# BosonHBC/BHRayTracer

Hardware: AMD Instinct MI355X
Metric: Mrays/s (closest-hit + any-hit rays per second), with wall-clock per frame (higher is better)
Workload: dtype f32

## Files before the change

bhraytracer_amd/csrc/device_state.h:

```cpp
#pragma once

namespace bhrt {

template <class T> struct DevBuf {
    T *p = nullptr;
    size_t n = 0;
    DevBuf() = default;
    DevBuf(const DevBuf &) = delete;
    DevBuf &operator=(const DevBuf &) = delete;
    DevBuf(DevBuf &&o) noexcept : p(o.p), n(o.n) { o.p = nullptr; o.n = 0; }
    DevBuf &operator=(DevBuf &&o) noexcept
    {
        if (this != &o) { Free(); p = o.p; n = o.n; o.p = nullptr; o.n = 0; }
        return *this;
    }
    ~DevBuf() { Free(); }
    int Reserve(size_t want)
    {
        if (n >= want) return BHRT_OK;
        Free();
        HIP_CHECK(hipMalloc(&p, want * sizeof(T)));
        n = want;
        return BHRT_OK;
    }
// ... 88 lines not shown
    int photon_exact = 0;
    uint32_t *d_knn = nullptr;
    DevBuf<uint32_t> d_sel;
    struct PendingTimer { int e0, e1; double *acc; };
    std::vector<PendingTimer> ev_pending;
    std::vector<int> ev_free;
    DevBuf<DPhoton> d_photons;
    uint32_t n_photons = 0;
    std::vector<HostPhoton> h_photons;
    DevBuf<float> d_ph_frames;
    DevBuf<float4> d_ph_hot, d_ph_cold, d_ph_dbox;
    PhotonMapDev pm;
    DevBuf<unsigned long long> d_scr;
    uint32_t scr_lanes = 0;
    uint32_t heavy_cap = 0;
    DevBuf<uint32_t> d_heavy;
    DevBuf<uint32_t> d_long;
    DevBuf<uint32_t> d_cell_of, d_gorder, d_rank_of, d_keys_out;
    DevBuf<uint8_t> d_sort_temp;
    size_t sort_temp_bytes = 0;
    DevBuf<uint32_t> d_n_heavy;
    PinnedBuf<uint32_t> h_n_heavy;
    DevBuf<uint32_t> d_cells, d_tile_sums;
    struct Knobs {
        int stream_waves = -1;
        bool fused_camera = true;
        bool no_slow_queue = false;
        bool debug_slow = false, debug_gather = false, debug_drain = false;
        bool balance_host = false;
        int frame_cap = 0;
        int gather_lane_budget = 0;
        bool gather_counting_sort = false;
        bool shadow_overlap = true;
        int gather_stats = 0;
        void FromEnv()
        {
            if (const char *e = getenv("BHRT_STREAM_WAVES")) stream_waves = atoi(e);
            if (const char *e = getenv("BHRT_FUSED_CAMERA")) fused_camera = atoi(e) != 0;
            no_slow_queue = getenv("BHRT_NO_SLOW_QUEUE") != nullptr;
            debug_slow = getenv("BHRT_DEBUG_SLOW") != nullptr; debug_gather = getenv("BHRT_DEBUG_GATHER") != nullptr; debug_drain = getenv("BHRT_DEBUG_DRAIN") != nullptr;
            if (const char *e = getenv("BHRT_PHOTON_BALANCE_HOST")) balance_host = atoi(e) != 0;
            if (const char *e = getenv("BHRT_GATHER_COUNTING_SORT")) gather_counting_sort = atoi(e) != 0;
            if (const char *e = getenv("BHRT_SHADOW_OVERLAP")) shadow_overlap = atoi(e) != 0;
        }
    } knobs;
    uint64_t pass_hint_key = 0;
    uint32_t pass_hint = 0;
    uint64_t frames_seen_key = 0;
    double frames_seen = 0;
    size_t frame_px = 0;
    DevBuf<uint8_t> d_frame_rgb;
    DevBuf<float> d_frame_rad, d_frame_var;
    DevBuf<uint32_t> d_frame_cnt;
    DevBuf<uint8_t> d_ad;
    DevBuf<uint8_t> d_dn;
    size_t api_cap = 0;
    DevBuf<float> d_api_f;
    DevBuf<int32_t> d_api_i;
};

void DestroyDeviceState(DeviceState *d)
{
    if (!d) return;
    if (d->device >= 0) (void)hipSetDevice(d->device);
    delete d;
}

}
```

bhraytracer_amd/csrc/kernels.hip:

```cpp
#include <hip/hip_runtime.h>

#include <stdlib.h>
#include <string.h>

#include <algorithm>
#include <type_traits>
#include <chrono>
#include <string>
#include <vector>

#include "bhrt.h"
#include "denoise.h"
#include "device_color24.h"
#include "device_photon.h"
#include "photon_host.h"
#include "scene_internal.h"

namespace bhrt {

#define HIP_CHECK(expr)                                                                                        \
    do {                                                                                                       \
        hipError_t e_ = (expr);                                                                                \
        if (e_ != hipSuccess) {                                                                                \
            SetError(std::string(#expr) + ": " + hipGetErrorString(e_));                                       \
// ... 183 lines not shown
{
    const uint32_t lane = __lane_id();
    const uint64_t lt = (1ull << lane) - 1ull;
    const uint64_t m0 = __ballot(cls == RC_HEAVY), m1 = __ballot(cls == RC_MEDIUM), m2 = __ballot(cls == RC_LIGHT), m3 = __ballot(cls == RC_MESH);
    uint32_t base = 0;
    if (lane < 4) {
        const uint64_t mk = lane == 0 ? m0 : (lane == 1 ? m1 : (lane == 2 ? m2 : m3));
        const uint32_t c = (uint32_t)__popcll(mk);
        if (c) base = atomicAdd(&cnt->cls[lane][shard].v, c);
    }
    const uint32_t wshard = shard;
    const uint32_t b0 = __shfl(base, 0), b1 = __shfl(base, 1), b2 = __shfl(base, 2), b3 = __shfl(base, 3);
    if (cls != RC_NONE) {
        const uint64_t mm = cls == RC_HEAVY ? m0 : (cls == RC_MEDIUM ? m1 : (cls == RC_LIGHT ? m2 : m3));
        const uint32_t pos = (cls == RC_HEAVY ? b0 : (cls == RC_MEDIUM ? b1 : (cls == RC_LIGHT ? b2 : b3))) + (uint32_t)__popcll(mm & lt);
        if (pos < ord.shard_cap) ord.idx[((size_t)cls * BHRT_ORDER_SHARDS + wshard) * ord.shard_cap + pos] = i;
        else atomicOr(&cnt->overflow.v, 8u);
    }
}
__device__ inline uint32_t shading_class(uint32_t meta, const Hit &hit)
{
    const uint32_t kind = meta & 15u;
    const bool is_hit = hit.node >= 0;
    bool heavy = false;
    if (is_hit) {
        if (kind == RK_CAMERA) heavy = true;
        else if (kind == RK_GI) heavy = fabsf(hit.t) > BHRT_BIAS;
        else if (kind == RK_REFR_IN) heavy = hit.front != 0;
        else heavy = true;
    }
    return heavy ? RC_HEAVY : ((kind == RK_REFR_IN && is_hit) ? RC_MEDIUM : RC_LIGHT);
}

struct SlowQueue {
    RayQueue q;
    uint32_t cap;
};
constexpr uint32_t kSlowCap = 1u << 16;
template <bool kPark, bool kCamera, bool kMeshes = true>
__global__ void __launch_bounds__(kBlock) k_trace_closest(DevScene S, PassInfo P, RayQueue q, uint32_t n, int uniform_side, HitBuf h, RayOrder ord, Counters *cnt,
                                                          SlowQueue slow )
{
    __shared__ bhrt_bvh_node nodelet[(kPark || !kMeshes) ? 1 : BHRT_LDS_NODES];
    const uint32_t i = blockIdx.x * blockDim.x + threadIdx.x;
    bool active = i < n;
    V3 o = v3(0, 0, 0), d = v3(0, 0, 1);
    uint32_t meta = 0;
    if (active) fetch_ray<kCamera>(S, P, q, i, o, d, meta);
    const bool has_meta = kCamera || q.meta;
    const int side = has_meta ? (int)((meta >> 4) & 3u) : uniform_side;
    const bool dead = has_meta && (meta & 15u) == RK_DEAD;
    Hit hit;
    uint32_t key = 0;
    bool is_slow = false;
    int parked = trace_closest<kMeshes>(S, o, d, side, hit, active && !dead, (kPark || !kMeshes) ? nullptr : nodelet, 0, kPark, kPark ? &key : nullptr,
                                        (uint16_t *)nullptr, 0, BHRT_LDS_NODES, kCamera, kPark ? &is_slow : nullptr);
    if (kPark && parked >= 0 && is_slow && slow.cap) {
        const uint32_t k = atomicAdd(&cnt->n_slow.v, 1u);
        if (k < slow.cap) {
            slow.q.ox[k] = o.x; slow.q.oy[k] = o.y; slow.q.oz[k] = o.z; slow.q.dx[k] = d.x; slow.q.dy[k] = d.y; slow.q.dz[k] = d.z;
            slow.q.frame[k] = kCamera ? i : q.frame[i];
            slow.q.meta[k] = meta;
            slow.q.rng_ctr[k] = (kCamera || (meta & 15u) == RK_GI) ? 0u : q.rng_ctr[i];
            active = false;
            parked = -1;
        }
    }
    if (active) { h.t[i] = hit.t; h.node[i] = hit.node; h.prim[i] = hit.prim; h.front[i] = hit.front | ((parked + 1) << 8); }
    if (kPark && parked >= 0) {
        ord.park_key[i] = key;
        if (!kCamera) ord.park_rank[i] = atomicAdd(&ord.park_bucket[key], 1u);
    }
    if (!ord.idx) return;
    uint32_t cls = RC_NONE;
    if (active && !dead) cls = parked >= 0 ? (uint32_t)RC_MESH : shading_class(meta, hit);
    file_ray(cls, i, (i >> 10) & (BHRT_ORDER_SHARDS - 1) , ord, cnt);
}
__device__ inline bool parked_entry(const RayOrder &ord, uint32_t b, uint32_t *s_seg, uint32_t &i, uint32_t first_entry = 0 )
{
    __syncthreads();
    if (threadIdx.x < 64) {
        const uint32_t l = threadIdx.x;
        const uint32_t a = l <= BHRT_ORDER_SHARDS ? ord.mesh_start[l] : 0xffffffffu;
        const uint32_t n_le = (uint32_t)__popcll(__ballot(l < BHRT_ORDER_SHARDS && a <= b));
        if (l == 0) *s_seg = n_le - 1;
    }
    __syncthreads();
    if (b >= ord.mesh_start[BHRT_ORDER_SHARDS]) return false;
    const uint32_t seg = *s_seg;
    const uint32_t local = (b - ord.mesh_start[seg]) * kBlock + first_entry + threadIdx.x;
    const bool active = local < ord.mesh_count[seg];
    i = active ? ord.idx[((size_t)RC_MESH * BHRT_ORDER_SHARDS + seg) * ord.shard_cap + local] : 0xffffffffu;
    return true;
}
#ifndef BHRT_XCD_LOCAL
#define BHRT_XCD_LOCAL 0
#endif
__device__ inline bool xcd_slice(uint32_t b, uint32_t nb, uint32_t &slice)
{
    slice = b;
#if BHRT_XCD_LOCAL
    constexpr uint32_t G = BHRT_XCD_LOCAL, span = 8 * G;
    const uint32_t chunk = b / span, in = b % span;
    if ((chunk + 1) * span <= nb) slice = chunk * span + (in & 7u) * G + (in >> 3);
#endif
    return b < nb;
}
__global__ void __launch_bounds__(kBlock) k_park_scatter(RayOrder ord)
{
    __shared__ uint32_t s_seg;
    uint32_t i;
    for (uint32_t b = blockIdx.x; parked_entry(ord, b, &s_seg, i); b += gridDim.x)
        if (i != 0xffffffffu) ord.park_sorted[ord.park_bucket[ord.park_key[i]] + ord.park_rank[i]] = i;
}
constexpr uint32_t kMeshNodelet = 256;
#ifndef BHRT_MESH_BLOCK
#define BHRT_MESH_BLOCK 64
#endif
constexpr int kMeshBlock = BHRT_MESH_BLOCK;
template <bool kCamera, int kPath, bool kLS = false>
__global__ void __launch_bounds__(kCamera ? kBlock : kMeshBlock, kPath == 1 ? 6 : 4 ) k_trace_mesh(DevScene S, PassInfo P, RayQueue q, HitBuf h, RayOrder ord, Counters *cnt)
{
    typedef typename std::conditional<kPath == 2, uint32_t, uint16_t>::type PathT;
    constexpr int kTB = kCamera ? kBlock : kMeshBlock;
    __shared__ bhrt_bvh_node nodelet[kPath ? 1 : kMeshNodelet];
    __shared__ PathT path[kPath ? 33 * kTB : 1];
    __shared__ uint32_t s_seg;
    bool active;
    uint32_t i;
    uint32_t slice;
    if (kCamera) {
        if (!xcd_slice(blockIdx.x, ord.mesh_start[BHRT_ORDER_SHARDS], slice)) return;
        if (!parked_entry(ord, slice, &s_seg, i)) return;
        active = i != 0xffffffffu;
        if (!active) i = 0;
    } else {
        const uint32_t total = ord.mesh_count[BHRT_ORDER_SHARDS];
        if (!xcd_slice(blockIdx.x, (total + kTB - 1) / kTB, slice)) return;
        const uint32_t k = slice * kTB + threadIdx.x;
        active = k < total;
        i = active ? ord.park_sorted[k] : 0u;
    }
    V3 o = v3(0, 0, 0), d = v3(0, 0, 1);
    uint32_t meta = 0;
    Hit hit = {BHRT_BIGFLOAT, -1, -1, 1};
    int start = 0;
    if (active) {
        fetch_ray<kCamera>(S, P, q, i, o, d, meta);
        hit.t = h.t[i]; hit.node = h.node[i]; hit.prim = h.prim[i];
        const int fw = h.front[i];
        hit.front = fw & 0xff;
        start = (fw >> 8) - 1;
    }
    trace_closest<true, PathT, kLS>(S, o, d, (int)((meta >> 4) & 3u), hit, active, kPath ? nullptr : nodelet, active ? start : S.n_nodes, false, nullptr,
                               kPath ? path + threadIdx.x : (PathT *)nullptr, kTB, kMeshNodelet);
    if (active) { h.t[i] = hit.t; h.node[i] = hit.node; h.prim[i] = hit.prim; h.front[i] = hit.front; }
    if (kCamera) file_ray(active ? shading_class(meta, hit) : (uint32_t)RC_NONE, i, slice & (BHRT_ORDER_SHARDS - 1), ord, cnt);
}
#ifndef BHRT_STREAM_REFILL
#define BHRT_STREAM_REFILL 32
#endif
constexpr int kStreamRefill = BHRT_STREAM_REFILL;
#ifndef BHRT_STREAM_OCC
#define BHRT_STREAM_OCC 6
#endif
#ifdef BHRT_DEBUG_DRAIN
__device__ unsigned long long g_stream_t[4];
#endif
#ifdef BHRT_DEBUG_STREAM
__device__ unsigned long long g_stream_dbg[8];
#endif
template <int kPath, bool kLS = false>
__global__ void __launch_bounds__(64, kPath == 1 ? BHRT_STREAM_OCC : (BHRT_STREAM_OCC < 5 ? BHRT_STREAM_OCC : 5) ) k_trace_mesh_stream(DevScene S, RayQueue q, HitBuf h, RayOrder ord, Counters *cnt)
{
    typedef typename std::conditional<kPath == 2, uint32_t, uint16_t>::type PathT;
    __shared__ PathT path[33 * 64];
    const uint32_t total = ord.mesh_count[BHRT_ORDER_SHARDS];
    const uint32_t lane = threadIdx.x;
    PathT *stack = path + lane;
    bool have = false, pending = false, exhausted = false;
    uint32_t i = 0;
    int n = 0, side = 0;
    Hit hit = {BHRT_BIGFLOAT, -1, -1, 1};
    MeshWalk W = {};
    W.st = 3;
    int cur_n = -1;
    MeshRef M = mesh_ref(S, 0);
#ifdef BHRT_DEBUG_STREAM
// ... 71 lines not shown
#endif
        for (;;) {
            const int nD = __popcll(__ballot(W.st == 0)), nL = __popcll(__ballot(W.st == 1)), nC = __popcll(__ballot(W.st == 2));
            const int walking = nD + nL + nC;
            if (walking == 0 || (!exhausted && 64 - walking - n_wait >= kStreamRefill)) break;
#ifdef BHRT_DEBUG_STREAM
#if BHRT_FUSED_CLIMB
            dbg[0]++; dbg[1] += walking; dbg[2] += (nD >= nL && nD > 0) ? nD : nL;
            if (nD >= nL && nD > 0) dbg[6]++; else if (nL > 0) dbg[7]++;
#else
            dbg[0]++; dbg[1] += walking; dbg[2] += (nD >= nL && nD >= nC) ? nD : (nL >= nC ? nL : nC);
            if (nD >= nL && nD >= nC) dbg[6]++; else if (nL >= nC) dbg[7]++;
#endif
#endif
#ifdef BHRT_DEBUG_STREAM
            const unsigned long long r0 = __builtin_readcyclecounter();
#endif
            walk_round<PathT, kLS>(M, W, side, hit.t, hit.prim, hit.front, stack, 64u, nD, nL, nC);
#ifdef BHRT_DEBUG_STREAM
            if (nD >= nL && nD > 0) dbg[4] += __builtin_readcyclecounter() - r0;
#endif
        }
#ifdef BHRT_DEBUG_STREAM
        { const unsigned long long c = __builtin_readcyclecounter(); dbg[3] += c - c_mark; c_mark = c; }
#endif
    }
#ifdef BHRT_DEBUG_STREAM
    if (lane == 0) for (int k = 0; k < 8; k++) atomicAdd(&g_stream_dbg[k], dbg[k]);
#endif
#ifdef BHRT_DEBUG_DRAIN
    if (lane == 0) atomicMax(&g_stream_t[2], wall_clock64());
#endif
}
__global__ void __launch_bounds__(kBlock) k_file_parked(RayQueue q, HitBuf h, RayOrder ord, Counters *cnt)
{
    __shared__ uint32_t s_seg;
    uint32_t i;
    if (!parked_entry(ord, blockIdx.x, &s_seg, i)) return;
    const bool active = i != 0xffffffffu;
    uint32_t cls = RC_NONE;
    if (active) {
        Hit hit;
        hit.t = h.t[i]; hit.node = h.node[i]; hit.prim = h.prim[i]; hit.front = h.front[i];
        cls = shading_class(q.meta[i], hit);
    }
    file_ray(cls, active ? i : 0u, blockIdx.x & (BHRT_ORDER_SHARDS - 1), ord, cnt);
}

__global__ void __launch_bounds__(64) k_trace_slow(DevScene S, SlowQueue slow, uint32_t a, uint32_t b, HitBuf h)
{
    __shared__ CoopLds lds;
    __builtin_amdgcn_s_setprio(3);
    const uint32_t i = a + blockIdx.x;
    if (i >= b) return;
    const V3 o = v3(slow.q.ox[i], slow.q.oy[i], slow.q.oz[i]), d = v3(slow.q.dx[i], slow.q.dy[i], slow.q.dz[i]);
    const uint32_t meta = slow.q.meta[i];
    Hit hit;
#ifdef BHRT_DEBUG_LONG_RAYS
    const unsigned long long c0 = wall_clock64();
#endif
    trace_closest_coop(S, lds, o, d, (int)((meta >> 4) & 3u), hit);
#ifdef BHRT_DEBUG_LONG_RAYS
    const double ms = (double)(wall_clock64() - c0) / 1e5;
    if (threadIdx.x == 0 && ms > 5.0) printf("slow ray %u: %.1f ms o=(%.9g %.9g %.9g) d=(%.9g %.9g %.9g) side %u -> node %d prim %d t %.9g\n", i, ms, o.x, o.y, o.z, d.x, d.y, d.z, (meta >> 4) & 3u, hit.node, hit.prim, hit.t);
#endif
    if (threadIdx.x == 0) { h.t[i] = hit.t; h.node[i] = hit.node; h.prim[i] = hit.prim; h.front[i] = hit.front; }
}
__global__ void __launch_bounds__(kBlock) k_inject_slow(RayQueue sq, HitBuf sh, uint32_t src0, uint32_t m, RayQueue q, HitBuf h, uint32_t dst0)
{
    const uint32_t k = blockIdx.x * blockDim.x + threadIdx.x;
    if (k >= m) return;
    const uint32_t a = src0 + k, b = dst0 + k;
    q.ox[b] = sq.ox[a]; q.oy[b] = sq.oy[a]; q.oz[b] = sq.oz[a]; q.dx[b] = sq.dx[a]; q.dy[b] = sq.dy[a]; q.dz[b] = sq.dz[a];
    q.frame[b] = sq.frame[a]; q.meta[b] = sq.meta[a]; q.rng_ctr[b] = sq.rng_ctr[a];
    h.t[b] = sh.t[a]; h.node[b] = sh.node[a]; h.prim[b] = sh.prim[a]; h.front[b] = sh.front[a];
}
static inline uint32_t kFileAllBlocks(uint32_t first, uint32_t n) { return (n - (first & ~63u) + kBlock - 1) / kBlock; }
// ... 332 lines not shown
            const uint64_t pcode = F.code[owner];
            skey = F.skey[owner];
            const uint32_t pi2 = F.info2[owner];
            gi = (int)(pi2 & 0xffu) - 64 - 1;
            if (kind == RK_GI) {
                code = pcode * 2 + 1;
                how = FH_GI;
                bounce = (int)((pi2 >> 8) & 0xffu);
            } else if (kind == RK_REFR_IN) {
                code = pcode * 2;
                how = FH_REFR_FRONT;
            } else {
                code = pcode * 2;
                how = FH_REFR_OUT;
                const bhrt_material &pm = S.materials[(F.info[owner] >> 20) & 0xfffu];
                V3 af = v3(dm::powf_(BHRT_EULER, -pm.absorption[0] * hit.t), dm::powf_(BHRT_EULER, -pm.absorption[1] * hit.t),
                           dm::powf_(BHRT_EULER, -pm.absorption[2] * hit.t));
                mult = ld3i(F.refr_color, owner) * af;
            }
        }
        F.parent[f] = owner;
        F.info2[f] = (uint32_t)(gi + 64) | ((uint32_t)(bounce & 0xff) << 8);
        F.skey[f] = skey;
        F.code[f] = code;
        if (how == FH_REFR_OUT) st3(F.mult, f, mult);
        const int mi = S.nodes[hit.node].material;
        const bool need_uv = kTex && mi >= 0 && (S.materials[mi].diffuse.map >= 0 || S.materials[mi].specular.map >= 0);
        Attr a;
        hit_attrs(S, o, d, hit.t, hit.node, hit.prim, need_uv, a);
        shade_entry<kTex>(S, R, F, f, how, o, a, hit.node, bounce, gi, code, skey, so);
        ray_owner = f;
    } else if (active) {
        if (kind == RK_CAMERA) {
            int pi, pj;
            uint32_t osmp;
            slot_pixel(P, owner, pi, pj, osmp);
            st3(samples, sample_addr(P, owner), kTex ? tc_sample(S, S.background, v3((float)pi / S.cam.width, (float)pj / S.cam.height, 0.0f)) : ld3(S.background.color));
        } else if (kind == RK_GI) {
            V3 mult = ld3i(F.gi_mult, owner);
            V3 outc = v3(0, 0, 0);
            if (is_hit) {
                outc = outc + v3(0, 0, 0) * mult;
            } else if (d.x == d.y && d.x == 0) {
                outc = outc + v3(1.0f, 0.0f, 1.0f);
            } else {
                V3 env = (kTex ? sample_environment(S, S.environment, d) : ld3(S.environment.color)) * mult;
                if (!(isnan_f(env.x) || isnan_f(env.y) || isnan_f(env.z))) outc = outc + env;
            }
            if (isnan_f(outc.x)) outc = v3(1.0f, 0.0f, 1.0f);
            else outc = clamp_white(outc);
            st3(F.gi, owner, outc);
        } else if (kind == RK_REFR_IN) {
            if (!is_hit) {
                st3(F.refr, owner, v3(1.0f, 0.0f, 1.0f));
            } else {
                Attr a;
                hit_attrs(S, o, d, hit.t, hit.node, hit.prim, false, a);
                const bhrt_material &m = S.materials[(F.info[owner] >> 20) & 0xfffu];
                const float refrGloss = m.glossiness > 50 ? m.glossiness : 0.f;
                V3 vN = a.N;
                V3 vV = -d;
                float cosPhi1 = dot(vV, -vN);
                float sinPhi1 = sqrtf(1 - cosPhi1 * cosPhi1);
                float sinPhi2 = m.ior * sinPhi1;
                if (sinPhi2 <= 1) {
                    float cosPhi2 = sqrtf(1 - sinPhi2 * sinPhi2);
                    V3 vTn = vN * cosPhi2;
                    V3 vNxV = cross(vN, vV);
                    V3 vTp = normalized(cross(vN, vNxV)) * sinPhi2;
                    V3 vT = vTn + vTp;
                    V3 vT_sampled = normalized(vT);
                    if (refrGloss > 0) {
                        DRng g;
                        g.key = bhrt_section_key(F.skey[owner], F.code[owner], BHRT_SEC_REFRACTION);
                        g.ctr = ctr;
                        float dotSign = 0;
                        int guard = 0;
                        while (dotSign <= 0 && guard++ < BHRT_MAXLOOP) {
                            float theta = 0;
                            vT_sampled = sample_along_light_direction(g, vT, refrGloss, theta);
                            dotSign = dot(vT_sampled, vN);
                        }
                        ctr = g.ctr;
                    }
// ... 1090 lines not shown
    while (q < n_items) {
        int rc = EnsureWorkspace(D, pass_samples, frames_per_sample);
        if (rc) return rc;
        R.cap_rays = D->cap_rays; R.cap_shadow = D->cap_rays; R.cap_frames = D->cap_frames;
        if (D->knobs.frame_cap > 0) R.cap_frames = std::min<uint32_t>(R.cap_frames, (uint32_t)D->knobs.frame_cap);
        if (o.photon_map) BHRT_TRY(D->d_ph_frames.Reserve((size_t)D->cap_frames * 15));
        if (pass_limit == 0) pass_limit = pass_samples;
        if (pass_limit > D->cap_samples) pass_limit = D->cap_samples;
        const uint32_t px_per_pass = pass_limit / spp;
        const uint32_t npx = (uint32_t)std::min<uint64_t>(px_per_pass, n_items - q);
        if (d_list) { P.list = d_list + q; P.q0 = 0; } else P.q0 = (uint32_t)q;
        P.n_pixels = npx;
        const bool sh_overlap = D->knobs.shadow_overlap && D->stream3 != nullptr && D->d_shf2.p != nullptr;
        const PassViews V = MakePassViews(D, sh_overlap);
        const Frames &F = V.F;
        const RayOrder &RO = V.RO;
        bool sh_pending[2] = {false, false};
        HIP_CHECK(hipMemsetAsync(D->d_cnt, 0, sizeof(Counters), D->stream));
        const uint32_t total = npx * spp;
        uint32_t n_cur = total;
        bool first_step = true;
        const bool lens = P.lens_r > 0.f;
        if (lens) {
            Timer t(D, &st->seconds_other);
            hipLaunchKernelGGL(k_lens_rays, dim3((total + kBlock - 1) / kBlock), dim3(kBlock), 0, D->stream, D->S, P, V.Q[0], total);
            t.Stop();
        }
        int cur = 0;
        std::vector<uint32_t> frame_marks = {0};
        bool overflow = false;
        uint64_t pass_closest = 0, pass_camera = 0, pass_shadow = 0, pass_deferred = 0;
        uint32_t pass_steps = 0;
        const SlowQueue no_slow = {V.slowq.q, 0u};
        uint32_t slow_pending = 0, slow_traced = 0, slow_injected = 0;
        struct SlowBatch { uint32_t end; uint32_t step; hipEvent_t done; };
        std::vector<SlowBatch> slow_batches;
        size_t slow_batch_next = 0;
#ifndef BHRT_INJECT_MIN_LOG2
#define BHRT_INJECT_MIN_LOG2 20
#endif
        constexpr uint32_t kInjectMinRays = 1u << BHRT_INJECT_MIN_LOG2;
        bool injected = false;
        if (D->stream2) HIP_CHECK(hipStreamSynchronize(D->stream2));
        if (D->stream3) HIP_CHECK(hipStreamSynchronize(D->stream3));
        int sh_wait_par = 0; uint32_t sh_wait_n = 0;
        auto launch_any_hit = [&](hipEvent_t after) -> int {
            if (!sh_wait_n) return BHRT_OK;
            const int par = sh_wait_par; const uint32_t n_sh = sh_wait_n;
            sh_wait_n = 0;
            HIP_CHECK(hipStreamWaitEvent(D->stream3, after, 0));
            LaunchAnyHit(D, D->stream3, H->n_meshes > 0, par ? V.SQ2 : V.SQ, n_sh, nullptr, F.vis, V.RO_sh, D->d_cnt_sh, path_mode, ls, &st->seconds_trace_shadow);
            HIP_CHECK(hipEventRecord(D->ev_shadow[par], D->stream3));
            sh_pending[par] = true;
            return BHRT_OK;
        };
        while (n_cur > 0 || slow_pending > slow_injected) {
            injected = false;
            uint32_t n_extra = 0;
            if (n_cur == 0) {
                const auto w0 = std::chrono::steady_clock::now();
                HIP_CHECK(hipStreamSynchronize(D->stream2));
                if (D->knobs.debug_slow)
                    fprintf(stderr, "slow rays: %u moved in after wave step %u, waited %.1f ms for their hits, pass time so far %.1f ms\n", slow_pending, pass_steps,
                            std::chrono::duration<double>(std::chrono::steady_clock::now() - w0).count() * 1e3, std::chrono::duration<double>(std::chrono::steady_clock::now() - wall0).count() * 1e3);
                n_cur = slow_pending - slow_injected;
                hipLaunchKernelGGL(k_inject_slow, dim3((n_cur + kBlock - 1) / kBlock), dim3(kBlock), 0, D->stream, V.slowq.q, V.slow_hits, slow_injected, n_cur, V.Q[cur], V.HB, 0u);
                pass_deferred += n_cur;
                slow_injected = slow_pending;
                slow_batch_next = slow_batches.size();
                injected = true;
            } else if (!first_step && n_cur >= kInjectMinRays) {
                uint32_t upto = slow_injected;
                size_t b = slow_batch_next;
                while (b < slow_batches.size() && slow_batches[b].step + 2 <= pass_steps) { upto = slow_batches[b].end; b++; }
                if (upto > slow_injected && (uint64_t)n_cur + (upto - slow_injected) <= D->cap_rays) {
                    HIP_CHECK(hipStreamWaitEvent(D->stream, slow_batches[b - 1].done, 0));
                    n_extra = upto - slow_injected;
                    hipLaunchKernelGGL(k_inject_slow, dim3((n_extra + kBlock - 1) / kBlock), dim3(kBlock), 0, D->stream, V.slowq.q, V.slow_hits, slow_injected, n_extra, V.Q[cur], V.HB, n_cur);
                    if (D->knobs.debug_slow) fprintf(stderr, "slow rays: %u ride along with wave step %u (%u rays)\n", n_extra, pass_steps, n_cur);
                    pass_deferred += n_extra;
                    slow_injected = upto;
                    slow_batch_next = b;
                }
            }
            const SlowQueue &sq = V.slowq;
            const bool cam_step = first_step && !lens;
            const bool fused = cam_step && H->n_meshes == 0 && D->knobs.fused_camera;
            if (fused) {
            } else if (injected) {
                Timer t(D, &st->seconds_trace_closest);
                hipLaunchKernelGGL(k_file_all, dim3((n_cur + kBlock - 1) / kBlock), dim3(kBlock), 0, D->stream, V.Q[cur], V.HB, 0u, n_cur, RO, D->d_cnt);
                t.Stop();
            } else {
                Timer t(D, &st->seconds_trace_closest);
                const dim3 tg((n_cur + kBlock - 1) / kBlock), tb(kBlock);
                if (H->n_meshes > 0) {
                    const uint32_t n_buckets = 1u << BHRT_PARK_KEY_BITS, n_tiles = n_buckets / kScanTile;
                    if (cam_step) hipLaunchKernelGGL(HIP_KERNEL_NAME(k_trace_closest<true, true>), tg, tb, 0, D->stream, D->S, P, V.Q[cur], n_cur, 0, V.HB, RO, D->d_cnt, sq);
                    else {
                        HIP_CHECK(hipMemsetAsync(RO.park_bucket, 0, n_buckets * sizeof(uint32_t), D->stream));
                        hipLaunchKernelGGL(HIP_KERNEL_NAME(k_trace_closest<true, false>), tg, tb, 0, D->stream, D->S, P, V.Q[cur], n_cur, 0, V.HB, RO, D->d_cnt, sq);
                    }
                    hipLaunchKernelGGL(k_mesh_prefix, dim3(1), dim3(64), 0, D->stream, D->d_cnt, RO);
                    if (!cam_step) {
                        const dim3 pg(std::min<uint32_t>(tg.x + BHRT_ORDER_SHARDS, 4096u));
                        hipLaunchKernelGGL(k_scan_tiles, dim3(n_tiles), dim3(kScanBlock), 0, D->stream, RO.park_bucket, n_buckets, RO.park_bucket + n_buckets);
                        hipLaunchKernelGGL(k_scan_sums, dim3(1), dim3(kScanBlock), 0, D->stream, RO.park_bucket + n_buckets, n_tiles);
                        hipLaunchKernelGGL(k_scan_add, dim3(n_tiles), dim3(kScanBlock), 0, D->stream, RO.park_bucket, n_buckets, RO.park_bucket + n_buckets);
                        hipLaunchKernelGGL(k_park_scatter, pg, tb, 0, D->stream, RO);
                    }
                    auto mesh_kernel = cam_step ? (path_mode == 1 ? (ls ? k_trace_mesh<true, 1, true> : k_trace_mesh<true, 1>) : path_mode == 2 ? (ls ? k_trace_mesh<true, 2, true> : k_trace_mesh<true, 2>) : k_trace_mesh<true, 0>)
                                                  : (path_mode == 1 ? k_trace_mesh<false, 1> : path_mode == 2 ? k_trace_mesh<false, 2> : k_trace_mesh<false, 0>);
                    if (sh_wait_n) {
                        HIP_CHECK(hipEventRecord(D->ev_shade, D->stream));
                        rc = launch_any_hit(D->ev_shade); if (rc) return rc;
                    }
                    if (!cam_step && path_mode != 0 && stream_waves > 0)
                    {
#ifdef BHRT_DEBUG_DRAIN
                        { unsigned long long t0[4] = {~0ull, ~0ull, 0, 0}; HIP_CHECK(hipMemcpyToSymbol(HIP_SYMBOL(g_stream_t), t0, sizeof(t0))); }
#endif
                        hipLaunchKernelGGL(path_mode == 1 ? (ls ? k_trace_mesh_stream<1, true> : k_trace_mesh_stream<1>) : (ls ? k_trace_mesh_stream<2, true> : k_trace_mesh_stream<2>), dim3(std::min<uint32_t>((n_cur + 63) / 64, stream_waves)), dim3(64), 0, D->stream, D->S,
                                           V.Q[cur], V.HB, RO, D->d_cnt);
#ifdef BHRT_DEBUG_DRAIN
                        unsigned long long t1[4];
                        HIP_CHECK(hipMemcpyFromSymbol(t1, HIP_SYMBOL(g_stream_t), sizeof(t1)));
                        static double dbg_total = 0, dbg_drain = 0;
                        if (t1[1] != ~0ull) { dbg_total += (double)(t1[2] - t1[0]) / 1e5; dbg_drain += (double)(t1[2] - t1[1]) / 1e5; }
                        if (D->knobs.debug_drain) fprintf(stderr, "mesh launch: %u rays, %.3f ms, of which %.3f ms after the list ran out (sums %.1f / %.1f ms)\n", n_cur, (double)(t1[2] - t1[0]) / 1e5, t1[1] != ~0ull ? (double)(t1[2] - t1[1]) / 1e5 : 0.0, dbg_total, dbg_drain);
#endif
                    }
                    else
                    hipLaunchKernelGGL(mesh_kernel, cam_step ? dim3(tg.x + BHRT_ORDER_SHARDS)  : dim3((n_cur + kMeshBlock - 1) / kMeshBlock),
                                       cam_step ? tb : dim3(kMeshBlock), 0, D->stream, D->S, P, V.Q[cur], V.HB, RO, D->d_cnt);
                    if (!cam_step) hipLaunchKernelGGL(k_file_parked, dim3(tg.x + BHRT_ORDER_SHARDS), tb, 0, D->stream, V.Q[cur], V.HB, RO, D->d_cnt);
                } else if (cam_step) hipLaunchKernelGGL(HIP_KERNEL_NAME(k_trace_closest<false, true, false>), tg, tb, 0, D->stream, D->S, P, V.Q[cur], n_cur, 0, V.HB, RO, D->d_cnt, no_slow);
                else hipLaunchKernelGGL(HIP_KERNEL_NAME(k_trace_closest<false, false, false>), tg, tb, 0, D->stream, D->S, P, V.Q[cur], n_cur, 0, V.HB, RO, D->d_cnt, no_slow);
                t.Stop();
            }
            if (n_extra) hipLaunchKernelGGL(k_file_all, dim3(kFileAllBlocks(n_cur, n_cur + n_extra)), dim3(kBlock), 0, D->stream, V.Q[cur], V.HB, n_cur, n_cur + n_extra, RO, D->d_cnt);
            if (!fused) {
                st->launches_trace_closest++;
                hipLaunchKernelGGL(k_order_prefix, dim3(1), dim3(128), 0, D->stream, D->d_cnt, RO);
            }
            const uint32_t seq = ++D->pub_seq;
            {
                Timer t(D, &st->seconds_shade, 0);
                const dim3 sg((n_cur + n_extra + kShadeBlock - 1) / kShadeBlock + (fused ? 0 : 3 * BHRT_ORDER_SHARDS)), sb(kShadeBlock);
                const bool tex = H->n_texmaps > 0;
                auto shade = fused ? (tex ? k_shade<true, true, true> : k_shade<true, false, true>)
                                   : cam_step ? (tex ? k_shade<true, true> : k_shade<true, false>) : (tex ? k_shade<false, true> : k_shade<false, false>);
                const int par = (int)(pass_steps & 1u);
                if (sh_wait_n) { HIP_CHECK(hipEventRecord(D->ev_shade, D->stream)); rc = launch_any_hit(D->ev_shade); if (rc) return rc; }
                if (sh_overlap && sh_pending[par]) { HIP_CHECK(hipStreamWaitEvent(D->stream, D->ev_shadow[par], 0)); sh_pending[par] = false; }
                hipLaunchKernelGGL(shade, sg, sb, 0, D->stream, D->S, R, P, V.Q[cur], V.HB, n_cur + n_extra, V.Q[cur ^ 1], (sh_overlap && par) ? V.SQ2 : V.SQ, F, D->d_samples, D->d_cnt, RO, D->d_pub, seq);
                t.Stop();
                if (sh_overlap) HIP_CHECK(hipEventRecord(D->ev_shade, D->stream));
            }
            if (!sh_overlap) {
                LaunchAnyHit(D, D->stream, H->n_meshes > 0, V.SQ, std::min<uint32_t>(n_cur + n_extra, R.cap_shadow), &D->d_cnt->n_shadow.v, F.vis, RO, D->d_cnt, path_mode, ls,
                             &st->seconds_trace_shadow);
            }
            rc = WaitPublished(D, seq);
            if (rc) return rc;
            const HostCounters hc = *D->h_pub;
            FlushTimers(D);
            if (hc.overflow) { overflow = true; break; }
            if (first_step) {
                const uint64_t valid_px = d_list ? npx : CountValidPixels(P, npx);
                pass_closest = valid_px * (uint64_t)spp;
// ... 201 lines not shown
        if (radiance) HIP_CHECK(hipMemcpyAsync(radiance, d_radiance, npix * 12, hipMemcpyDeviceToHost, s));
        if (variance) HIP_CHECK(hipMemcpyAsync(variance, d_variance, npix * 12, hipMemcpyDeviceToHost, s));
        if (count) HIP_CHECK(hipMemcpyAsync(count, d_count, npix * 4, hipMemcpyDeviceToHost, s));
        HIP_CHECK(hipStreamSynchronize(s));
        return BHRT_OK;
    }
};

}

using namespace bhrt;

extern "C" {

int bhrt_device_count(int *n)
try {
    if (!n) { SetError("null argument"); return BHRT_ERR_ARG; }
    int c = 0;
    hipError_t e = hipGetDeviceCount(&c);
    if (e != hipSuccess) { *n = 0; SetError(std::string("hipGetDeviceCount: ") + hipGetErrorString(e)); return BHRT_ERR_NO_DEVICE; }
    *n = c;
    return BHRT_OK;
} catch (...) { return bhrt::AbiException(); }

int bhrt_scene_knob(bhrt_scene *scene, const char *name, int value)
try {
    int rc = EnsureUploaded(scene);
    if (rc) return rc;
    if (!name || value < 0) { SetError("knob: bad arguments"); return BHRT_ERR_ARG; }
    if (!strcmp(name, "frame_cap")) scene->dev->knobs.frame_cap = value;
    else if (!strcmp(name, "gather_lane_budget")) scene->dev->knobs.gather_lane_budget = value;
    else if (!strcmp(name, "gather_stats")) scene->dev->knobs.gather_stats = value;
    else if (!strcmp(name, "shadow_overlap")) scene->dev->knobs.shadow_overlap = value != 0;
    else { SetError(std::string("knob: unknown name ") + name); return BHRT_ERR_ARG; }
    return BHRT_OK;
} catch (...) { return bhrt::AbiException(); }

int bhrt_scene_upload(bhrt_scene *scene, int device)
try {
    if (!scene) { SetError("null scene"); return BHRT_ERR_ARG; }
    if (scene->dev && scene->dev->device == device) { HIP_CHECK(hipSetDevice(device)); return BHRT_OK; }
    int count = 0;
    if (hipGetDeviceCount(&count) != hipSuccess || count <= 0) { SetError("no HIP device available (this path has no CPU fallback)"); return BHRT_ERR_NO_DEVICE; }
    if (device < 0 || device >= count) { SetError("device index out of range"); return BHRT_ERR_ARG; }
    if (scene->max_bvh_depth > 64) { SetError("BVH deeper than 64 levels: the stackless trail holds 64"); return BHRT_ERR_UNSUPPORTED; }
    if (scene->dev) { DestroyDeviceState(scene->dev); scene->dev = nullptr; }
    HIP_CHECK(hipSetDevice(device));
    DeviceState *D = new DeviceState;
    D->knobs.FromEnv();
    D->device = device;
    scene->dev = D;
    {
        int cus = 0;
        if (hipDeviceGetAttribute(&cus, hipDeviceAttributeMultiprocessorCount, device) == hipSuccess && cus > 0) D->n_cus = (uint32_t)cus;
    }
    const std::vector<uint8_t> &blob = scene->flat.blob;
    const bhrt_flat_header *H = scene->flat.hdr();
    HIP_CHECK(hipStreamCreate(&D->stream));
    HIP_CHECK(hipEventCreate(&D->ev[0]));
    HIP_CHECK(hipEventCreate(&D->ev[1]));
    BHRT_TRY(D->d_blob.Reserve(blob.size()));
    HIP_CHECK(hipMemcpy(D->d_blob, blob.data(), blob.size(), hipMemcpyHostToDevice));
    std::vector<int32_t> chain((size_t)std::max<uint32_t>(H->n_nodes, 1) * BHRT_MAX_NODE_DEPTH, 0);
    const bhrt_node *nodes = (const bhrt_node *)(blob.data() + H->off_nodes);
    for (uint32_t n = 0; n < H->n_nodes; n++) {
        int k = nodes[n].depth - 1, c = (int)n;
// ... 70 lines not shown
        float x = halton(i, 2), y = halton(i, 3);
        float r = sqrtf(x) * 0.5f;
        S.tapx[i] = r * dm::sinf_(y * (float)M_PI * 2);
        S.tapy[i] = r * dm::cosf_(y * (float)M_PI * 2);
        if (!(fabsf(S.tapx[i]) <= 0.5f && fabsf(S.tapy[i]) <= 0.5f)) { SetError("footprint tap outside the half-unit disc"); return BHRT_ERR_UNSUPPORTED; }
    }
    return BHRT_OK;
} catch (...) { return bhrt::AbiException(); }

static int EnsureApiScratch(DeviceState *D, size_t n)
{
    if (D->api_cap >= n) return BHRT_OK;
    D->api_cap = 0;
    BHRT_TRY(D->d_api_f.Reserve(n * 9));
    BHRT_TRY(D->d_api_i.Reserve(n * 3));
    D->api_cap = n;
    return BHRT_OK;
}

int bhrt_trace_closest_dev(bhrt_scene *scene, const float *d_rays_soa, int hit_side, size_t n, bhrt_hits d_out, void *stream)
try {
    int rc = EnsureUploaded(scene);
    if (rc) return rc;
    if (!d_rays_soa || !d_out.t || !d_out.node || !d_out.prim || !d_out.front) { SetError("null buffer"); return BHRT_ERR_ARG; }
    if (hit_side < 1 || hit_side > 3) { SetError("hit_side must be 1, 2 or 3"); return BHRT_ERR_ARG; }
    if (n == 0) return BHRT_OK;
    if (n > 0x7fffffffu) { SetError("too many rays for one call"); return BHRT_ERR_ARG; }
    RayQueue q = MakeRayQueue(const_cast<float *>(d_rays_soa), nullptr, n);
    HitBuf h; h.t = d_out.t; h.node = d_out.node; h.prim = d_out.prim; h.front = d_out.front;
    hipStream_t s = stream ? (hipStream_t)stream : scene->dev->stream;
    RayOrder no_order = {nullptr, 0, nullptr, nullptr, nullptr, nullptr, nullptr, nullptr, nullptr, nullptr};
    auto closest_kernel = scene->flat.hdr()->n_meshes > 0 ? k_trace_closest<false, false, true> : k_trace_closest<false, false, false>;
    hipLaunchKernelGGL(closest_kernel, dim3((unsigned)((n + kBlock - 1) / kBlock)), dim3(kBlock), 0, s,
                       scene->dev->S, PassInfo(), q, (uint32_t)n, hit_side, h, no_order, (Counters *)nullptr, SlowQueue{q, 0u});
    HIP_CHECK(hipGetLastError());
    if (!stream) HIP_CHECK(hipStreamSynchronize(s));
    return BHRT_OK;
} catch (...) { return bhrt::AbiException(); }

int bhrt_trace_closest_host(bhrt_scene *scene, const float *rays_soa, int hit_side, size_t n, bhrt_hits out)
try {
    int rc = EnsureUploaded(scene);
    if (rc) return rc;
    if (n == 0) return BHRT_OK;
    if (!rays_soa || !out.t || !out.node || !out.prim || !out.front) { SetError("null buffer"); return BHRT_ERR_ARG; }
    DeviceState *D = scene->dev;
    rc = EnsureApiScratch(D, n);
    if (rc) return rc;
    HIP_CHECK(hipMemcpy(D->d_api_f, rays_soa, n * 6 * sizeof(float), hipMemcpyHostToDevice));
    bhrt_hits d; d.t = D->d_api_f + 6 * n; d.node = D->d_api_i; d.prim = D->d_api_i + n; d.front = D->d_api_i + 2 * n;
    rc = bhrt_trace_closest_dev(scene, D->d_api_f, hit_side, n, d, nullptr);
    if (rc) return rc;
    HIP_CHECK(hipMemcpy(out.t, d.t, n * sizeof(float), hipMemcpyDeviceToHost));
    HIP_CHECK(hipMemcpy(out.node, d.node, n * sizeof(int32_t), hipMemcpyDeviceToHost));
    HIP_CHECK(hipMemcpy(out.prim, d.prim, n * sizeof(int32_t), hipMemcpyDeviceToHost));
    HIP_CHECK(hipMemcpy(out.front, d.front, n * sizeof(int32_t), hipMemcpyDeviceToHost));
    return BHRT_OK;
} catch (...) { return bhrt::AbiException(); }

int bhrt_trace_shadow_dev(bhrt_scene *scene, const float *d_rays_soa, const float *d_tmax, size_t n, float *d_vis, void *stream)
try {
    int rc = EnsureUploaded(scene);
    if (rc) return rc;
    if (!d_rays_soa || !d_tmax || !d_vis) { SetError("null buffer"); return BHRT_ERR_ARG; }
    if (n == 0) return BHRT_OK;
    if (n > 0x7fffffffu) { SetError("too many rays for one call"); return BHRT_ERR_ARG; }
    ShadowQueue q = MakeShadowQueue(const_cast<float *>(d_rays_soa), nullptr, n);
// ... 748 lines not shown
```

Measured before the change: 6612.

## Resolve camera and GI misses inside trace kernels instead of the shading pass

Camera rays and GI rays that miss all geometry now write their background or environment contribution directly in the closest-hit, mesh and parked-filing kernels, and are not filed into the shading order queues. This is meant to cut hit-buffer writes, queue filing and shading-kernel work for rays that need only a trivial lookup. It adds per-ray texture sampling and branching to the trace kernels, which can raise register pressure and lengthen divergent tails there. A knob (default on) selects whether parked mesh rays take the same path.

```diff
diff --git a/bhraytracer_amd/csrc/device_state.h b/bhraytracer_amd/csrc/device_state.h
--- a/bhraytracer_amd/csrc/device_state.h
+++ b/bhraytracer_amd/csrc/device_state.h
@@ -144,6 +144,7 @@
         int gather_lane_budget = 0;
         bool gather_counting_sort = false;
         bool shadow_overlap = true;
+        int miss_in_trace = 1;
         int gather_stats = 0;
         void FromEnv()
         {
@@ -154,6 +155,7 @@
             if (const char *e = getenv("BHRT_PHOTON_BALANCE_HOST")) balance_host = atoi(e) != 0;
             if (const char *e = getenv("BHRT_GATHER_COUNTING_SORT")) gather_counting_sort = atoi(e) != 0;
             if (const char *e = getenv("BHRT_SHADOW_OVERLAP")) shadow_overlap = atoi(e) != 0;
+            if (const char *e = getenv("BHRT_MISS_IN_TRACE")) { const int v = atoi(e); miss_in_trace = v < 0 || v > 2 ? 1 : v; }
         }
     } knobs;
     uint64_t pass_hint_key = 0;
diff --git a/bhraytracer_amd/csrc/kernels.hip b/bhraytracer_amd/csrc/kernels.hip
--- a/bhraytracer_amd/csrc/kernels.hip
+++ b/bhraytracer_amd/csrc/kernels.hip
@@ -239,6 +239,36 @@
     return heavy ? RC_HEAVY : ((kind == RK_REFR_IN && is_hit) ? RC_MEDIUM : RC_LIGHT);
 }
 
+struct MissSink {
+    float *samples;
+    float *gi;
+    const float *gi_mult;
+    int tex;
+};
+__device__ inline void camera_miss(const DevScene &S, const PassInfo &P, uint32_t slot, float *samples, bool tex)
+{
+    int pi, pj;
+    uint32_t osmp;
+    slot_pixel(P, slot, pi, pj, osmp);
+    st3(samples, sample_addr(P, slot), tex ? tc_sample(S, S.background, v3((float)pi / S.cam.width, (float)pj / S.cam.height, 0.0f)) : ld3(S.background.color));
+}
+__device__ inline void gi_miss(const DevScene &S, float *gi, const float *gi_mult, uint32_t owner, V3 d, bool is_hit, bool tex)
+{
+    V3 mult = ld3i(gi_mult, owner);
+    V3 outc = v3(0, 0, 0);
+    if (is_hit) {
+        outc = outc + v3(0, 0, 0) * mult;
+    } else if (d.x == d.y && d.x == 0) {
+        outc = outc + v3(1.0f, 0.0f, 1.0f);
+    } else {
+        V3 env = (tex ? sample_environment(S, S.environment, d) : ld3(S.environment.color)) * mult;
+        if (!(isnan_f(env.x) || isnan_f(env.y) || isnan_f(env.z))) outc = outc + env;
+    }
+    if (isnan_f(outc.x)) outc = v3(1.0f, 0.0f, 1.0f);
+    else outc = clamp_white(outc);
+    st3(gi, owner, outc);
+}
+
 struct SlowQueue {
     RayQueue q;
     uint32_t cap;
@@ -246,7 +276,7 @@
 constexpr uint32_t kSlowCap = 1u << 16;
 template <bool kPark, bool kCamera, bool kMeshes = true>
 __global__ void __launch_bounds__(kBlock) k_trace_closest(DevScene S, PassInfo P, RayQueue q, uint32_t n, int uniform_side, HitBuf h, RayOrder ord, Counters *cnt,
-                                                          SlowQueue slow )
+                                                          SlowQueue slow , MissSink miss)
 {
     __shared__ bhrt_bvh_node nodelet[(kPark || !kMeshes) ? 1 : BHRT_LDS_NODES];
     const uint32_t i = blockIdx.x * blockDim.x + threadIdx.x;
@@ -273,14 +303,20 @@
             parked = -1;
         }
     }
-    if (active) { h.t[i] = hit.t; h.node[i] = hit.node; h.prim[i] = hit.prim; h.front[i] = hit.front | ((parked + 1) << 8); }
+    bool finished = false;
+    if (active && !dead && parked < 0 && hit.node < 0) {
+        if (kCamera) {
+            if (miss.samples) { camera_miss(S, P, i, miss.samples, miss.tex != 0); finished = true; }
+        } else if (kPark && miss.gi && (meta & 15u) == RK_GI) { gi_miss(S, miss.gi, miss.gi_mult, q.frame[i], d, false, miss.tex != 0); finished = true; }
+    }
+    if (active && !finished) { h.t[i] = hit.t; h.node[i] = hit.node; h.prim[i] = hit.prim; h.front[i] = hit.front | ((parked + 1) << 8); }
     if (kPark && parked >= 0) {
         ord.park_key[i] = key;
         if (!kCamera) ord.park_rank[i] = atomicAdd(&ord.park_bucket[key], 1u);
     }
     if (!ord.idx) return;
     uint32_t cls = RC_NONE;
-    if (active && !dead) cls = parked >= 0 ? (uint32_t)RC_MESH : shading_class(meta, hit);
+    if (active && !dead && !finished) cls = parked >= 0 ? (uint32_t)RC_MESH : shading_class(meta, hit);
     file_ray(cls, i, (i >> 10) & (BHRT_ORDER_SHARDS - 1) , ord, cnt);
 }
 __device__ inline bool parked_entry(const RayOrder &ord, uint32_t b, uint32_t *s_seg, uint32_t &i, uint32_t first_entry = 0 )
@@ -326,7 +362,7 @@
 #endif
 constexpr int kMeshBlock = BHRT_MESH_BLOCK;
 template <bool kCamera, int kPath, bool kLS = false>
-__global__ void __launch_bounds__(kCamera ? kBlock : kMeshBlock, kPath == 1 ? 6 : 4 ) k_trace_mesh(DevScene S, PassInfo P, RayQueue q, HitBuf h, RayOrder ord, Counters *cnt)
+__global__ void __launch_bounds__(kCamera ? kBlock : kMeshBlock, kPath == 1 ? 6 : 4 ) k_trace_mesh(DevScene S, PassInfo P, RayQueue q, HitBuf h, RayOrder ord, Counters *cnt, MissSink miss)
 {
     typedef typename std::conditional<kPath == 2, uint32_t, uint16_t>::type PathT;
     constexpr int kTB = kCamera ? kBlock : kMeshBlock;
@@ -361,6 +397,10 @@
     }
     trace_closest<true, PathT, kLS>(S, o, d, (int)((meta >> 4) & 3u), hit, active, kPath ? nullptr : nodelet, active ? start : S.n_nodes, false, nullptr,
                                kPath ? path + threadIdx.x : (PathT *)nullptr, kTB, kMeshNodelet);
+    if (kCamera && active && hit.node < 0 && miss.samples) {
+        camera_miss(S, P, i, miss.samples, miss.tex != 0);
+        active = false;
+    }
     if (active) { h.t[i] = hit.t; h.node[i] = hit.node; h.prim[i] = hit.prim; h.front[i] = hit.front; }
     if (kCamera) file_ray(active ? shading_class(meta, hit) : (uint32_t)RC_NONE, i, slice & (BHRT_ORDER_SHARDS - 1), ord, cnt);
 }
@@ -498,7 +538,7 @@
     if (lane == 0) atomicMax(&g_stream_t[2], wall_clock64());
 #endif
 }
-__global__ void __launch_bounds__(kBlock) k_file_parked(RayQueue q, HitBuf h, RayOrder ord, Counters *cnt)
+__global__ void __launch_bounds__(kBlock) k_file_parked(DevScene S, RayQueue q, HitBuf h, RayOrder ord, Counters *cnt, MissSink miss)
 {
     __shared__ uint32_t s_seg;
     uint32_t i;
@@ -508,7 +548,12 @@
     if (active) {
         Hit hit;
         hit.t = h.t[i]; hit.node = h.node[i]; hit.prim = h.prim[i]; hit.front = h.front[i];
-        cls = shading_class(q.meta[i], hit);
+        const uint32_t meta = q.meta[i];
+        cls = shading_class(meta, hit);
+        if (miss.gi && hit.node < 0 && (meta & 15u) == RK_GI) {
+            gi_miss(S, miss.gi, miss.gi_mult, q.frame[i], v3(q.dx[i], q.dy[i], q.dz[i]), false, miss.tex != 0);
+            cls = RC_NONE;
+        }
     }
     file_ray(cls, active ? i : 0u, blockIdx.x & (BHRT_ORDER_SHARDS - 1), ord, cnt);
 }
@@ -907,24 +952,9 @@
         ray_owner = f;
     } else if (active) {
         if (kind == RK_CAMERA) {
-            int pi, pj;
-            uint32_t osmp;
-            slot_pixel(P, owner, pi, pj, osmp);
-            st3(samples, sample_addr(P, owner), kTex ? tc_sample(S, S.background, v3((float)pi / S.cam.width, (float)pj / S.cam.height, 0.0f)) : ld3(S.background.color));
+            camera_miss(S, P, owner, samples, kTex);
         } else if (kind == RK_GI) {
-            V3 mult = ld3i(F.gi_mult, owner);
-            V3 outc = v3(0, 0, 0);
-            if (is_hit) {
-                outc = outc + v3(0, 0, 0) * mult;
-            } else if (d.x == d.y && d.x == 0) {
-                outc = outc + v3(1.0f, 0.0f, 1.0f);
-            } else {
-                V3 env = (kTex ? sample_environment(S, S.environment, d) : ld3(S.environment.color)) * mult;
-                if (!(isnan_f(env.x) || isnan_f(env.y) || isnan_f(env.z))) outc = outc + env;
-            }
-            if (isnan_f(outc.x)) outc = v3(1.0f, 0.0f, 1.0f);
-            else outc = clamp_white(outc);
-            st3(F.gi, owner, outc);
+            gi_miss(S, F.gi, F.gi_mult, owner, d, is_hit, kTex);
         } else if (kind == RK_REFR_IN) {
             if (!is_hit) {
                 st3(F.refr, owner, v3(1.0f, 0.0f, 1.0f));
@@ -2081,6 +2111,9 @@
         uint64_t pass_closest = 0, pass_camera = 0, pass_shadow = 0, pass_deferred = 0;
         uint32_t pass_steps = 0;
         const SlowQueue no_slow = {V.slowq.q, 0u};
+        const MissSink no_miss = {nullptr, nullptr, nullptr, 0};
+        const MissSink miss = D->knobs.miss_in_trace ? MissSink{D->d_samples, F.gi, F.gi_mult, H->n_texmaps > 0 ? 1 : 0} : no_miss;
+        const MissSink miss_parked = D->knobs.miss_in_trace == 1 ? miss : no_miss;
         uint32_t slow_pending = 0, slow_traced = 0, slow_injected = 0;
         struct SlowBatch { uint32_t end; uint32_t step; hipEvent_t done; };
         std::vector<SlowBatch> slow_batches;
@@ -2145,10 +2178,10 @@
                 const dim3 tg((n_cur + kBlock - 1) / kBlock), tb(kBlock);
                 if (H->n_meshes > 0) {
                     const uint32_t n_buckets = 1u << BHRT_PARK_KEY_BITS, n_tiles = n_buckets / kScanTile;
-                    if (cam_step) hipLaunchKernelGGL(HIP_KERNEL_NAME(k_trace_closest<true, true>), tg, tb, 0, D->stream, D->S, P, V.Q[cur], n_cur, 0, V.HB, RO, D->d_cnt, sq);
+                    if (cam_step) hipLaunchKernelGGL(HIP_KERNEL_NAME(k_trace_closest<true, true>), tg, tb, 0, D->stream, D->S, P, V.Q[cur], n_cur, 0, V.HB, RO, D->d_cnt, sq, miss);
                     else {
                         HIP_CHECK(hipMemsetAsync(RO.park_bucket, 0, n_buckets * sizeof(uint32_t), D->stream));
-                        hipLaunchKernelGGL(HIP_KERNEL_NAME(k_trace_closest<true, false>), tg, tb, 0, D->stream, D->S, P, V.Q[cur], n_cur, 0, V.HB, RO, D->d_cnt, sq);
+                        hipLaunchKernelGGL(HIP_KERNEL_NAME(k_trace_closest<true, false>), tg, tb, 0, D->stream, D->S, P, V.Q[cur], n_cur, 0, V.HB, RO, D->d_cnt, sq, miss);
                     }
                     hipLaunchKernelGGL(k_mesh_prefix, dim3(1), dim3(64), 0, D->stream, D->d_cnt, RO);
                     if (!cam_step) {
@@ -2181,10 +2214,10 @@
                     }
                     else
                     hipLaunchKernelGGL(mesh_kernel, cam_step ? dim3(tg.x + BHRT_ORDER_SHARDS)  : dim3((n_cur + kMeshBlock - 1) / kMeshBlock),
-                                       cam_step ? tb : dim3(kMeshBlock), 0, D->stream, D->S, P, V.Q[cur], V.HB, RO, D->d_cnt);
-                    if (!cam_step) hipLaunchKernelGGL(k_file_parked, dim3(tg.x + BHRT_ORDER_SHARDS), tb, 0, D->stream, V.Q[cur], V.HB, RO, D->d_cnt);
-                } else if (cam_step) hipLaunchKernelGGL(HIP_KERNEL_NAME(k_trace_closest<false, true, false>), tg, tb, 0, D->stream, D->S, P, V.Q[cur], n_cur, 0, V.HB, RO, D->d_cnt, no_slow);
-                else hipLaunchKernelGGL(HIP_KERNEL_NAME(k_trace_closest<false, false, false>), tg, tb, 0, D->stream, D->S, P, V.Q[cur], n_cur, 0, V.HB, RO, D->d_cnt, no_slow);
+                                       cam_step ? tb : dim3(kMeshBlock), 0, D->stream, D->S, P, V.Q[cur], V.HB, RO, D->d_cnt, miss);
+                    if (!cam_step) hipLaunchKernelGGL(k_file_parked, dim3(tg.x + BHRT_ORDER_SHARDS), tb, 0, D->stream, D->S, V.Q[cur], V.HB, RO, D->d_cnt, miss_parked);
+                } else if (cam_step) hipLaunchKernelGGL(HIP_KERNEL_NAME(k_trace_closest<false, true, false>), tg, tb, 0, D->stream, D->S, P, V.Q[cur], n_cur, 0, V.HB, RO, D->d_cnt, no_slow, miss);
+                else hipLaunchKernelGGL(HIP_KERNEL_NAME(k_trace_closest<false, false, false>), tg, tb, 0, D->stream, D->S, P, V.Q[cur], n_cur, 0, V.HB, RO, D->d_cnt, no_slow, miss);
                 t.Stop();
             }
             if (n_extra) hipLaunchKernelGGL(k_file_all, dim3(kFileAllBlocks(n_cur, n_cur + n_extra)), dim3(kBlock), 0, D->stream, V.Q[cur], V.HB, n_cur, n_cur + n_extra, RO, D->d_cnt);
@@ -2452,6 +2485,7 @@
     else if (!strcmp(name, "gather_lane_budget")) scene->dev->knobs.gather_lane_budget = value;
     else if (!strcmp(name, "gather_stats")) scene->dev->knobs.gather_stats = value;
     else if (!strcmp(name, "shadow_overlap")) scene->dev->knobs.shadow_overlap = value != 0;
+    else if (!strcmp(name, "miss_in_trace")) scene->dev->knobs.miss_in_trace = value > 2 ? 1 : value;
     else { SetError(std::string("knob: unknown name ") + name); return BHRT_ERR_ARG; }
     return BHRT_OK;
 } catch (...) { return bhrt::AbiException(); }
@@ -2588,7 +2622,7 @@
     RayOrder no_order = {nullptr, 0, nullptr, nullptr, nullptr, nullptr, nullptr, nullptr, nullptr, nullptr};
     auto closest_kernel = scene->flat.hdr()->n_meshes > 0 ? k_trace_closest<false, false, true> : k_trace_closest<false, false, false>;
     hipLaunchKernelGGL(closest_kernel, dim3((unsigned)((n + kBlock - 1) / kBlock)), dim3(kBlock), 0, s,
-                       scene->dev->S, PassInfo(), q, (uint32_t)n, hit_side, h, no_order, (Counters *)nullptr, SlowQueue{q, 0u});
+                       scene->dev->S, PassInfo(), q, (uint32_t)n, hit_side, h, no_order, (Counters *)nullptr, SlowQueue{q, 0u}, MissSink{nullptr, nullptr, nullptr, 0});
     HIP_CHECK(hipGetLastError());
     if (!stream) HIP_CHECK(hipStreamSynchronize(s));
     return BHRT_OK;
```

Measured after the change: 6580. No clear change (-0.5%).
